# gopro/cineform-sdk

Measured on AMD Instinct MI355X. Metric: 1080p YUY2 encode+decode fps, higher is better.
Workload: dtype int16

## Files before the change

cineform-sdk_amd/csrc/cfhd_device.hip:

```cpp
#include "cfhd_device.h"
#include "cfhd_kernels.h"
#include "cfhd_collect_kernels.h"
#include <hip/hip_runtime.h>
#include <string.h>
#include <stddef.h>
#include <vector>
#include <stdlib.h>
#include <stdio.h>
#include <mutex>
#include <thread>
#include <atomic>
#include <string>
#include <utility>

namespace cfhd {

namespace {
std::string g_err_text; std::mutex g_err_mutex;
thread_local std::string t_err_copy;
struct ErrSlot { ErrSlot &operator=(const char *t) { std::lock_guard<std::mutex> l(g_err_mutex); g_err_text = t; return *this; } } g_err;
std::once_flag g_init_once;
int g_init_rc = -1;
int g_device = 0;

// ... 564 lines not shown
		if (pitch == in_pitch_) memcpy(dst + off, src + (size_t)r0 * pitch, bytes);
		else for (int r = r0; r < r1; r++) memcpy(dst + (size_t)r * in_pitch_, src + (size_t)r * pitch, (size_t)in_pitch_);
		HIPCHK(hipMemcpyAsync(d_in_ + frame_bytes_ * i + off, dst + off, bytes, hipMemcpyHostToDevice, (hipStream_t)stream_));
	}
	return 0;
}

int EncodeBatch::upload_frames(const void *frames, size_t frame_stride, int pitch)
{
	(void)hipSetDevice(device_);
	if (!frames) return -1;
	if (plan_.pixel_kind == PIX_AV28 && pitch >= 0) pitch = in_pitch_;
	if (pitch == in_pitch_ && frame_stride == frame_bytes_ && plan_.pixel_kind != PIX_BYR4 && plan_.pixel_kind != PIX_BYR5 && host_buffer_is_registered(frames, frame_bytes_ * (size_t)n_)) {
		HIPCHK(hipMemcpyAsync(d_in_, frames, frame_bytes_ * (size_t)n_, hipMemcpyHostToDevice, (hipStream_t)stream_));
		return 0;
	}
	if (n_ > 8 && pitch >= in_pitch_ && plan_.pixel_kind != PIX_BYR4 && plan_.pixel_kind != PIX_BYR5 && !host_buffer_is_registered(frames, 1)) {
		const int nt = n_ < 8 ? n_ : 8;
		std::atomic<int> next(0);
		auto work = [&] {
			for (int i; (i = next.fetch_add(1)) < n_;) {
				const uint8_t *src = (const uint8_t *)frames + frame_stride * (size_t)i; uint8_t *dst = h_in_ + frame_bytes_ * (size_t)i;
				if (pitch == in_pitch_) memcpy(dst, src, frame_bytes_);
				else for (int r = 0; r < in_rows_; r++) memcpy(dst + (size_t)r * in_pitch_, src + (size_t)r * pitch, (size_t)in_pitch_);
			}
		};
		std::vector<std::thread> pool;
		for (int k = 1; k < nt; k++) pool.emplace_back(work);
		work();
		for (auto &t : pool) t.join();
		HIPCHK(hipMemcpyAsync(d_in_, h_in_, frame_bytes_ * (size_t)n_, hipMemcpyHostToDevice, (hipStream_t)stream_));
		return 0;
	}
	for (int i = 0; i < n_; i++) { const int rc = upload_frame(i, (const uint8_t *)frames + frame_stride * (size_t)i, pitch); if (rc) return rc; }
	return 0;
}

static double frames_1080p_equivalent(const FramePlan &plan, int frames) { return (double)frames * plan.width * plan.height / (1920.0 * 1080.0); }
static int shape_override(const char *name)
{
	const char *e = getenv(name);
	return !e ? 0 : (strcmp(e, "tile") == 0 ? 1 : (strcmp(e, "strip") == 0 ? 2 : 0));
}
static int active_frames(int active, int n) { return active > 0 && active < n ? active : n; }
static bool planes_as_strips(const FramePlan &plan, int lv , int frames)
{
	const int forced = shape_override("CFHD_AMD_PLANES");
	double samples = 0.0;
	for (int c = 0; c < plan.num_channels; c++) samples += (double)plan.ch[c].width * plan.ch[c].height;
	if (forced == 1 || (forced == 0 && frames * samples / (2.0 * 1920.0 * 1080.0) < 160.0)) return false;
	for (int c = 0; c < plan.num_channels; c++) {
		const BandDesc &b = plan.ch[c].band[lv][0];
		if (b.width % dev::SBLK || plan.ch[c].band[lv - 1][0].width != 2 * b.width || plan.ch[c].band[lv - 1][0].height != 2 * b.height ||
		    (plan.ch[c].band[lv - 1][0].pitch & 7) || (b.pitch & 7)) return false;
	}
	return true;
}
template <typename F> static void for_channel_runs(const FramePlan &plan, int lv, F f)
{
	for (int c0 = 0; c0 < plan.num_channels;) {
		int nc = 1;
		while (c0 + nc < plan.num_channels && plan.ch[c0 + nc].band[lv][0].width == plan.ch[c0].band[lv][0].width &&
		       plan.ch[c0 + nc].band[lv][0].height == plan.ch[c0].band[lv][0].height) nc++;
		const BandDesc &b = plan.ch[c0].band[lv][0];
		int glog = 0; while ((1 << glog) < b.width / dev::SBLK) glog++;
		const int nblk = b.width / dev::SBLK, nseg = nblk > 64 ? (nblk + dev::PLSTEP - 1) / dev::PLSTEP : 1;
		if (nseg > 1) glog = 6;
		f(c0, nc, glog, b, nseg);
		c0 += nc;
	}
}

struct PlaneStrips { int nstrips; unsigned blocks; };
static PlaneStrips plane_strips(int frames, int nc, int glog, int nseg, int band_height)
{
	const int nstrips = (band_height + dev::SRP - 1) / dev::SRP, per_wave = nseg > 1 ? 1 : 64 >> glog, waves = ((frames * nc + per_wave - 1) / per_wave) * nstrips * nseg;
	return { nstrips, (unsigned)((waves + 3) / 4) };
}
static void launch_fwd_plane_tiles(const dev::FwdPlaneJob *jobs, int width, int height, int planes, hipStream_t st) { dev::k_fwd_plane<<<dim3((width / 2 + dev::TW - 1) / dev::TW, (height / 2 + dev::TH - 1) / dev::TH, planes), dev::NTHREADS, 0, st>>>(jobs); }

enum class FwdL1 { Yuv422, Yuv422Strip, Yuv422StripBlocks, Yuv422StripBlocksDense, FrameYuv422, FrameYuv422Strip, Packed16, Packed16Strip, BayerStrip, BayerUnpack, GopPacked16 };
static const char *const kFwdL1Name[] = {"k_fwd_yuv422", "k_fwd_yuv422_strip", "k_fwd_yuv422_strip_blocks", "k_fwd_yuv422_strip_blocks_dense", "k_fwd_frame_yuv422",
                                         "k_fwd_frame_yuv422_strip", "k_fwd_packed16", "k_fwd_packed16_strip", "k_fwd_bayer_strip", "k_unpack_byr4+k_fwd_plane", "k_fwd_gop_packed16"};
static const char *const kFwdPlaneName[2] = {"k_fwd_plane", "k_fwd_plane_strip"};
static_assert(sizeof(kFwdL1Name) / sizeof(*kFwdL1Name) == (size_t)FwdL1::GopPacked16 + 1, "one name per level-1 kernel");
struct ForwardRoute {
	FwdL1 l1; bool strip_planes[2];
	bool block_lists() const { return l1 == FwdL1::Yuv422StripBlocks || l1 == FwdL1::Yuv422StripBlocksDense; }
};
template <typename F> static bool every_frame(int n, F ok) { for (int i = 0; i < n; i++) if (!ok(i)) return false; return true; }

ForwardRoute EncodeBatch::forward_route(bool coeffs_needed, int frames) const
{
	static const int blocks_env = [] { const char *e = getenv("CFHD_AMD_BLOCKS"); return e ? atoi(e) : 1; }();
	const int act = frames, forced = shape_override("CFHD_AMD_FORWARD"), kind = plan_.pixel_kind, nch = plan_.num_channels;
	const EncJobs j = enc_jobs_at(h_jobs_, n_, nch);
	ForwardRoute r;
	for (int lv = 1; lv < 3; lv++) r.strip_planes[lv - 1] = planes_as_strips(plan_, lv, act);
	const bool strips = forced != 1 && (forced != 0 || frames_1080p_equivalent(plan_, act) >= 32.0);
	const bool yuy2 = kind == PIX_YUY2 || kind == PIX_2VUY, bayer = kind == PIX_BYR4 || kind == PIX_BYR5;
	const bool yuv_strips = strips && plan_.encoded_format == ENC_YUV422 && plan_.width % 32 == 0 &&
	                        every_frame(n_, [&](int i) { return !((uintptr_t)j.yuv[i].in & 15) && !(j.yuv[i].in_pitch & 15); });
	if (bayer) {
		const bool ok = strips && kind == PIX_BYR4 && plan_.width % 8 == 0 && nch == 4 &&
		                every_frame(n_, [&](int i) { return !((uintptr_t)j.bayer[i].in & 15) && !((j.bayer[i].in_pitch * 2) & 15) && j.bayer[i].order == j.bayer[0].order; });
		r.l1 = ok ? FwdL1::BayerStrip : FwdL1::BayerUnpack;
	} else if (strips && is_packed16(kind) && plan_.encoded_format != ENC_YUV422 && plan_.width % 8 == 0 && nch >= 3 && every_frame(n_, [&](int i) {
		const dev::FwdPlaneJob &p = j.l1[(size_t)i * nch];
		const uintptr_t frame = (uintptr_t)((const uint16_t *)p.in - packed_word_of_channel(kind, 0));
		return !(frame & 15) && !((p.in_pitch * 2) & 15) && p.layout == dev::FWD_WORDS16 && p.width % 8 == 0; })) r.l1 = FwdL1::Packed16Strip;
	else if (enc_packed16(kind)) r.l1 = FwdL1::Packed16;
	else if (plan_.interlaced) r.l1 = yuv_strips && yuy2 ? FwdL1::FrameYuv422Strip : FwdL1::FrameYuv422;
	else if (!yuv_strips) r.l1 = FwdL1::Yuv422;
	else if (blocks_env && ent_ready_ && ent_.block_slots() && yuy2) r.l1 = coeffs_needed ? FwdL1::Yuv422StripBlocksDense : FwdL1::Yuv422StripBlocks;
	else r.l1 = FwdL1::Yuv422Strip;
	return r;
}

struct FirstLevel {
	int width, height, frames;
	const dev::FwdYuvJob *yuv; const dev::FwdPlaneJob *l1; const dev::BayerJob *bayer;
	int nch, pixel_kind;
	int luma_tiles, chroma_tiles;
};
static int launch_first_level(FwdL1 k, const FirstLevel &g, hipStream_t st)
{
	static_assert(sizeof(dev::FwdFrameJob) == sizeof(dev::FwdYuvJob) && offsetof(dev::FwdFrameJob, q) == offsetof(dev::FwdYuvJob, q), "the two level-1 jobs share one table");
	const int hw = g.width / 2, hh = g.height / 2, act = g.frames, nch = g.nch;
	const dim3 tiles((hw + dev::TW - 1) / dev::TW, (hh + dev::TH - 1) / dev::TH, act);
	auto strips422 = [&](int rows) { return dim3((g.width / 16 + dev::SSEG - 1) / dev::SSEG, (hh + rows - 1) / rows, act); };
	const int nseg = (g.width / 8 + dev::PSTEP - 1) / dev::PSTEP, nstrips = (hh + dev::PSR - 1) / dev::PSR, waves = act * nseg * nstrips;
	const dev::FwdFrameJob *frame = (const dev::FwdFrameJob *)g.yuv;
	const bool bayer = k == FwdL1::BayerStrip || k == FwdL1::BayerUnpack, planes = bayer || k == FwdL1::Packed16 || k == FwdL1::Packed16Strip || k == FwdL1::GopPacked16;
	if ((planes ? !g.l1 : !g.yuv) || (bayer && !g.bayer)) { g_err = "forward level 1: no job table for the kernel"; return -1; }
	switch (k) {
	case FwdL1::Packed16: dev::k_fwd_packed16<<<dim3(tiles.x * nch, tiles.y, act), dev::NTHREADS, 0, st>>>(g.l1, nch); break;
	case FwdL1::GopPacked16: dev::k_fwd_gop_packed16<<<dim3(g.luma_tiles + 2 * g.chroma_tiles, tiles.y, act), dev::NTHREADS, 0, st>>>(g.l1, g.luma_tiles); break;
	case FwdL1::BayerStrip: dev::k_fwd_bayer_strip<<<(waves + 3) / 4, dev::NTHREADS, 0, st>>>(g.l1, g.bayer, act, nseg, nstrips); break;
	case FwdL1::BayerUnpack:
		dev::k_unpack_byr4<<<dim3((hw + dev::NTHREADS - 1) / dev::NTHREADS, g.height, act), dev::NTHREADS, 0, st>>>(g.bayer);
		launch_fwd_plane_tiles(g.l1, g.width, g.height, act * nch, st);
		break;
	case FwdL1::Packed16Strip:
		if (g.pixel_kind == PIX_RG48) dev::k_fwd_packed16_strip<3, 3><<<dim3((waves + 3) / 4), dev::NTHREADS, 0, st>>>(g.l1, act, nseg, nstrips);
		else if (nch == 4) dev::k_fwd_packed16_strip<4, 4><<<dim3((waves + 3) / 4), dev::NTHREADS, 0, st>>>(g.l1, act, nseg, nstrips);
		else dev::k_fwd_packed16_strip<4, 3><<<dim3((waves + 3) / 4), dev::NTHREADS, 0, st>>>(g.l1, act, nseg, nstrips);
		break;
	case FwdL1::FrameYuv422Strip: dev::k_fwd_frame_yuv422_strip<<<strips422(dev::SRI), dev::NTHREADS, 0, st>>>(frame); break;
	case FwdL1::FrameYuv422: dev::k_fwd_frame_yuv422<<<dim3((hw + dev::FTW - 1) / dev::FTW, (hh + dev::FRW - 1) / dev::FRW, act), dev::NTHREADS, 0, st>>>(frame); break;
	case FwdL1::Yuv422StripBlocksDense: dev::k_fwd_yuv422_strip_blocks_dense<<<strips422(dev::SRF), dev::NTHREADS, 0, st>>>(g.yuv); break;
	case FwdL1::Yuv422StripBlocks: dev::k_fwd_yuv422_strip_blocks<<<strips422(dev::SRF), dev::NTHREADS, 0, st>>>(g.yuv); break;
	case FwdL1::Yuv422Strip: dev::k_fwd_yuv422_strip<<<strips422(dev::SRF), dev::NTHREADS, 0, st>>>(g.yuv); break;
	case FwdL1::Yuv422: dev::k_fwd_yuv422<<<tiles, dev::NTHREADS, 0, st>>>(g.yuv); break;
	}
	return 0;
}

const char *EncodeBatch::level_kernel(int level, bool coeffs_needed) const
{
	const ForwardRoute r = forward_route(coeffs_needed, active_frames(active_, n_));
	return level > 0 ? kFwdPlaneName[r.strip_planes[level - 1]] : kFwdL1Name[(int)r.l1];
}

int EncodeBatch::launch_forward(bool coeffs_needed, int first, int count)
{
	if (!count) count = active_frames(active_, n_);
	if (first < 0 || count < 1 || first + count > n_) return -1;
	(void)hipSetDevice(device_);
	const ForwardRoute r = forward_route(coeffs_needed, count);
	if (ent_ready_) ent_.set_block_lists(r.block_lists());
	int rc = sync_jobs();
	if (rc) return rc;
	hipStream_t st = (hipStream_t)stream_;
	const int nch = plan_.num_channels;
	const int act = count;
	EncJobs j = enc_jobs_at(d_jobs_, n_, nch);
	if (j.yuv) j.yuv += first;
	if (j.bayer) j.bayer += first;
	if (j.l1) j.l1 += (size_t)first * nch;
	j.l2 += (size_t)first * nch; j.l3 += (size_t)first * nch;
	(void)hipGetLastError();
	timed_ = true;
	HIPCHK(hipEventRecord((hipEvent_t)ev0_, st));
	rc = launch_first_level(r.l1, { plan_.width, plan_.height, act, j.yuv, j.l1, j.bayer, nch, plan_.pixel_kind, 0, 0 }, st);
	if (rc) return rc;
	for (int lv = 1; lv < 3; lv++) {
		HIPCHK(hipEventRecord((hipEvent_t)evl_[lv - 1], st));
		const BandDesc &src = plan_.ch[0].band[lv - 1][0];
		const dev::FwdPlaneJob *jobs = lv == 1 ? j.l2 : j.l3;
		if (r.strip_planes[lv - 1]) {
			for_channel_runs(plan_, lv, [&](int c0, int nc, int glog, const BandDesc &b, int nseg) {
				const PlaneStrips g = plane_strips(act, nc, glog, nseg, b.height);
				dev::k_fwd_plane_strip<<<g.blocks, dev::NTHREADS, 0, st>>>(jobs, act, nch, c0, nc, glog, g.nstrips, 2 * b.width, 2 * b.height, nseg);
			});
			continue;
		}
		launch_fwd_plane_tiles(jobs, src.width, src.height, act * nch, st);
	}
	HIPCHK(hipGetLastError());
	HIPCHK(hipEventRecord((hipEvent_t)ev1_, st));
	return 0;
}

int EncodeBatch::download_coeffs()
{
	(void)hipSetDevice(device_);
	HIPCHK(hipMemcpy2DAsync(h_coeff_, (size_t)plan_.final_elems * 2, d_coeff_, (size_t)plan_.coeff_elems * 2,
	                        (size_t)plan_.final_elems * 2, n_, hipMemcpyDeviceToHost, (hipStream_t)stream_));
	return 0;
}

int EncodeBatch::wait()
{
	(void)hipSetDevice(device_);
	HIPCHK(hipStreamSynchronize((hipStream_t)stream_));
	collect_.resolve();
	float ms = 0;
	if (!timed_) return 0;
	timed_ = false;
	if (hipEventElapsedTime(&ms, (hipEvent_t)ev0_, (hipEvent_t)ev1_) == hipSuccess) kernel_ms_ = ms;
	if (hipEventElapsedTime(&ms, (hipEvent_t)ev0_, (hipEvent_t)evl_[0]) == hipSuccess) level_ms_[0] = ms;
	if (hipEventElapsedTime(&ms, (hipEvent_t)evl_[0], (hipEvent_t)evl_[1]) == hipSuccess) level_ms_[1] = ms;
	if (hipEventElapsedTime(&ms, (hipEvent_t)evl_[1], (hipEvent_t)ev1_) == hipSuccess) level_ms_[2] = ms;
	return 0;
}

static OutputRoute output_route(int encoded_format, int kind, bool half, bool interlaced)
{
	OutputRoute r; r.work = kind; r.lowpass_kind = kind;
	const bool yuv8 = kind == PIX_YUY2 || kind == PIX_2VUY, rgb32 = kind == PIX_BGRA || kind == PIX_BGRa, rgb16 = is_packed16(kind), rgb8 = dec_rgb8(kind), rgb10 = dec_rgb10(kind);
	auto refuse = [&r](const char *text) { r.refusal = text; return r; };
	static const char *const not_served = "output format not supported by the GPU path yet";
	if (kind == PIX_BYR4) {
		if (encoded_format != ENC_BAYER || half) return refuse("BYR4 output: Bayer samples, full resolution");
		r.jobs = OutJobs::Planes16; r.work = PIX_RG48; r.convert = OutConvert::Byr4;
		return r;
	}
	if (encoded_format == ENC_YUV422) {
		if (!yuv8 && kind != PIX_YU64 && kind != PIX_V210 && !rgb8 && !rgb16) return refuse(not_served);
		if (kind == PIX_V210) { r.work = PIX_YU64; r.convert = OutConvert::V210; r.width_multiple = 6; r.width_refusal = "v210 output: widths that are multiples of 6"; }
		if (half) {
			r.jobs = OutJobs::HalfYuv;
			if (rgb8 || rgb16) { r.half_mode = kind == PIX_RG24 ? 0 : (kind == PIX_RG48 ? 2 : (kind == PIX_B64A ? 3 : 1)); r.bottom_up = kind == PIX_BGRA; }
			if (rgb32) { r.width_multiple = 16; r.width_refusal = "BGRA / BGRa output of 4:2:2 samples: half widths that are multiples of 16"; }
			return r;
		}
		if (yuv8) return r;
		if (rgb32 && !interlaced) return r;
		r.work = PIX_YU64;
		r.jobs = interlaced && (rgb16 || rgb32) ? OutJobs::Yuv : OutJobs::Planes16;
		if (kind == PIX_RG24) r.convert = OutConvert::Rgb24;
		if (rgb16 || rgb32) { r.convert = OutConvert::Rgb16; r.rgb16_mode = kind == PIX_BGRA ? 3 : (kind == PIX_BGRa ? 2 : (kind == PIX_B64A ? 1 : 0)); }
		return r;
	}
	const bool rgb = encoded_format == ENC_RGB444, rgba = encoded_format == ENC_RGBA4444;
	if (!((rgb16 && (rgb || rgba)) || (rgb8 && (rgb || (rgba && kind != PIX_RG24))) || (rgb10 && rgb))) return refuse(not_served);
	if (!half) { r.jobs = OutJobs::Planes16; return r; }
	r.jobs = OutJobs::HalfPacked;
	if (rgb8 || rgb10 || (kind == PIX_B64A && rgb)) {
		r.half_mode = rgb8 ? 1 : (rgb10 ? 2 : 3); r.half_bytes = rgb8 ? rgb8_bytes(kind) : 0;
		r.bottom_up = kind == PIX_RG24 || kind == PIX_BGRA; r.big_endian = kind == PIX_R210 || kind == PIX_DPX0;
	}
	return r;
}

static void fill_half_yuv_job(dev::HalfYuvJob &hj, const Level1 &l, const OutputRoute &r, int rows, int matrix, uint8_t *out, int out_pitch)
{
// ... 764 lines not shown
		g = e;
	}
	return 0;
}

int GopBatch::upload_frame(int f, const void *frame, int pitch)
{
	(void)hipSetDevice(device_);
	if (decode_ || f < 0 || f >= 2 * n_) return -1;
	const uint8_t *src = (const uint8_t *)frame;
	const bool av28 = plan_.pixel_kind == PIX_AV28;
	if (pitch < 0) { src += (ptrdiff_t)(rows_ - 1) * pitch; pitch = -pitch; }
	uint8_t *dst = h_frames_ + frame_bytes_ * f;
	if (pitch == pitch_ || av28) memcpy(dst, src, frame_bytes_);
	else for (int r = 0; r < rows_; r++) memcpy(dst + (size_t)r * pitch_, src + (size_t)r * pitch, (size_t)pitch_);
	HIPCHK(hipMemcpyAsync(d_frames_ + frame_bytes_ * f, dst, frame_bytes_, hipMemcpyHostToDevice, (hipStream_t)stream_));
	return 0;
}

int GopBatch::upload_frame_device(int f, const void *d_frame, int pitch)
{
	(void)hipSetDevice(device_);
	if (decode_ || f < 0 || f >= 2 * n_ || !d_frame) return -1;
	const uint8_t *src = (const uint8_t *)d_frame;
	if (pitch < 0) { src += (ptrdiff_t)(rows_ - 1) * pitch; pitch = -pitch; }
	if (plan_.pixel_kind == PIX_AV28) {
		HIPCHK(hipMemcpyAsync(d_frames_ + frame_bytes_ * f, src, frame_bytes_, hipMemcpyDeviceToDevice, (hipStream_t)stream_));
		return 0;
	}
	if (pitch < pitch_) return -1;
	HIPCHK(hipMemcpy2DAsync(d_frames_ + frame_bytes_ * f, (size_t)pitch_, src, (size_t)pitch, (size_t)pitch_, (size_t)rows_, hipMemcpyDeviceToDevice, (hipStream_t)stream_));
	return 0;
}

int GopBatch::upload_frames_device_planar(int first, int count, const void *d_frames, size_t frame_stride, int row_pitch, int layout)
{
	(void)hipSetDevice(device_);
	if (decode_) return -1;
	return collect_planar_frames(plan_.pixel_kind, d_frames_, frame_bytes_, pitch_, plan_.width, rows_, 2 * n_, first, count, d_frames, frame_stride, row_pitch, layout, stream_, collect_);
}

int GopBatch::download_input_frame(int f, void *out, int pitch)
{
	(void)hipSetDevice(device_);
	const size_t row = pitch_ ? (size_t)pitch_ : frame_bytes_, nrows = pitch_ ? (size_t)rows_ : 1;
	if (decode_ || f < 0 || f >= 2 * n_ || !out || pitch < 0 || (size_t)pitch < row) return -1;
	HIPCHK(hipMemcpy2DAsync(out, (size_t)pitch, d_frames_ + frame_bytes_ * f, row, row, nrows, hipMemcpyDeviceToHost, (hipStream_t)stream_));
	HIPCHK(hipStreamSynchronize((hipStream_t)stream_));
	return 0;
}

int GopBatch::upload_frames(const void *frames, size_t frame_stride, int pitch)
{
	(void)hipSetDevice(device_);
	if (decode_ || !frames || pitch <= 0) return -1;
	const size_t total = 2 * (size_t)n_ * frame_bytes_;
	const bool av28 = plan_.pixel_kind == PIX_AV28;
	if ((pitch == pitch_ || av28) && frame_stride == frame_bytes_ && host_buffer_is_registered(frames, total)) {
		HIPCHK(hipMemcpyAsync(d_frames_, frames, total, hipMemcpyHostToDevice, (hipStream_t)stream_));
		return 0;
	}
	for (int f = 0; f < 2 * n_; f++) {
		const uint8_t *src = (const uint8_t *)frames + frame_stride * (size_t)f;
		uint8_t *dst = h_frames_ + frame_bytes_ * f;
		if (pitch == pitch_ || av28) memcpy(dst, src, frame_bytes_);
		else for (int r = 0; r < rows_; r++) memcpy(dst + (size_t)r * pitch_, src + (size_t)r * pitch, (size_t)(pitch < pitch_ ? pitch : pitch_));
	}
	HIPCHK(hipMemcpyAsync(d_frames_, h_frames_, total, hipMemcpyHostToDevice, (hipStream_t)stream_));
	return 0;
}

int GopBatch::launch_forward(int first, int count)
{
	if (first < 0 || count < 1 || first + count > n_) return -1;
	(void)hipSetDevice(device_);
	hipStream_t st = (hipStream_t)stream_;
	const int rcj = sync_jobs();
	if (rcj) return rcj;
	GopJobs j = gop_jobs_at(d_jobs_, n_);
	j.yuv += 2 * first; j.fl1 += 6 * first; j.temp += 3 * first; j.mid += 6 * first; j.top += 3 * first; j.tq += 3 * first;
	(void)hipGetLastError();
	if (timed_) HIPCHK(hipEventRecord((hipEvent_t)ev_[0], st));
	const int luma_tiles = (plan_.ch[0].width / 2 + dev::TW - 1) / dev::TW, chroma_tiles = (plan_.ch[1].width / 2 + dev::TW - 1) / dev::TW;
	const int rc = launch_first_level(forward_route(), { plan_.width, plan_.height, 2 * count, j.yuv, j.fl1, nullptr, 3, plan_.pixel_kind, luma_tiles, chroma_tiles }, st);
	if (rc) return rc;
	if (timed_) HIPCHK(hipEventRecord((hipEvent_t)ev_[1], st));
	const GopWavelet &t = plan_.ch[0].w[2];
	dev::k_gop_temporal_fwd<<<dim3((unsigned)((t.pitch * t.height / 2 + dev::NTHREADS - 1) / dev::NTHREADS), 3 * count), dev::NTHREADS, 0, st>>>(j.temp);
	launch_fwd_plane_tiles(j.mid, t.width, t.height, 6 * count, st);
	if (!decode_ && gop_temporal_lowpass_is_coded(plan_)) {
		const GopWavelet &w3 = plan_.ch[0].w[3];
		dev::k_gop_quant_lowpass<<<dim3((unsigned)((w3.pitch * w3.height / 2 + dev::NTHREADS - 1) / dev::NTHREADS), 3 * count), dev::NTHREADS, 0, st>>>(j.tq);
	}
	if (timed_) HIPCHK(hipEventRecord((hipEvent_t)ev_[2], st));
	const GopWavelet &m = plan_.ch[0].w[4];
	launch_fwd_plane_tiles(j.top, m.width, m.height, 3 * count, st);
	HIPCHK(hipGetLastError());
	if (timed_) { HIPCHK(hipEventRecord((hipEvent_t)ev_[3], st)); launched_ = true; }
	return 0;
}

int GopBatch::download_coeffs()
{
	(void)hipSetDevice(device_);
	HIPCHK(hipMemcpyAsync(h_coeff_, d_coeff_, plan_.coeff_elems * 2, hipMemcpyDeviceToHost, (hipStream_t)stream_));
	return 0;
}

int GopBatch::launch_inverse(uint32_t dither_seed, bool coeffs_on_device)
{
	(void)hipSetDevice(device_);
	hipStream_t st = (hipStream_t)stream_;
	if (jobs_dirty_) { HIPCHK(hipMemcpyAsync(d_jobs_, h_jobs_, jobs_bytes_, hipMemcpyHostToDevice, st)); jobs_dirty_ = false; }
	if (!coeffs_on_device) HIPCHK(hipMemcpyAsync(d_coeff_, h_coeff_, plan_.coeff_elems * 2, hipMemcpyHostToDevice, st));
	if (!coeffs_on_device && n_ != 1) return -1;
	GopJobs j = gop_jobs_at(d_jobs_, n_);
	const int ng = active_groups();
	(void)hipGetLastError();
	if (timed_) HIPCHK(hipEventRecord((hipEvent_t)ev_[0], st));
	const GopWavelet &top = plan_.ch[0].w[5], &mid = plan_.ch[0].w[4], &t = plan_.ch[0].w[2], &l1 = plan_.ch[0].w[0];
	dev::k_inv_plane<<<dim3((top.width + dev::ITW - 1) / dev::ITW, (top.height + dev::ITH - 1) / dev::ITH, 3 * ng), dev::NTHREADS, 0, st>>>(j.itop);
	if (timed_) HIPCHK(hipEventRecord((hipEvent_t)ev_[1], st));
	dev::k_inv_plane<<<dim3((mid.width + dev::ITW - 1) / dev::ITW, (mid.height + dev::ITH - 1) / dev::ITH, 6 * ng), dev::NTHREADS, 0, st>>>(j.imid);
	dev::k_gop_temporal_inv<<<dim3((unsigned)((t.pitch * t.height / 2 + dev::NTHREADS - 1) / dev::NTHREADS), 3 * ng), dev::NTHREADS, 0, st>>>(j.temp);
	if (timed_) HIPCHK(hipEventRecord((hipEvent_t)ev_[2], st));
	const GopRoute r = route();
	const int rc = launch_last_level(r.l1, { l1.width, l1.height, rows_, 2 * ng, plan_.interlaced, j.iyuv, j.l1, j.half, nullptr, 3, dec_words_per_position(PIX_YU64, 3) }, dither_seed, st);
	if (rc) return rc;
	auto convert = [&](int f, int nf, size_t step, int m) {
		launch_convert(r.out, d_tmp_ + tmp_frame_bytes_ * f, tmp_pitch_, tmp_frame_bytes_ * step, d_frames_ + frame_bytes_ * f, pitch_, frame_bytes_ * step, half_ ? plan_.width / 2 : plan_.width, rows_, 0, nf, m,
		               dither_seed + 0x9E3779B9u * (uint32_t)f, nullptr, st);
	};
	if (matrix_ == 0 || r.out.convert == OutConvert::V210) convert(0, 2 * ng, 1, 0); else { convert(0, ng, 2, matrix_); convert(1, ng, 2, 0); }
	HIPCHK(hipGetLastError());
	if (timed_) { HIPCHK(hipEventRecord((hipEvent_t)ev_[3], st)); launched_ = true; }
	return 0;
}

int GopBatch::download_frame(int f, void *, int)
{
	(void)hipSetDevice(device_);
	if (!decode_ || f < 0 || f >= 2 * n_) return -1;
	HIPCHK(hipMemcpyAsync(h_frames_ + frame_bytes_ * f, d_frames_ + frame_bytes_ * f, frame_bytes_, hipMemcpyDeviceToHost, (hipStream_t)stream_));
	return 0;
}

int GopBatch::download_frames(void *out, size_t, int pitch)
{
	(void)hipSetDevice(device_);
	if (!decode_ || !out || pitch <= 0) return -1;
	HIPCHK(hipMemcpyAsync(h_frames_, d_frames_, 2 * (size_t)active_groups() * frame_bytes_, hipMemcpyDeviceToHost, (hipStream_t)stream_));
	return 0;
}

int GopBatch::finish_frame(int f, void *out, int pitch)
{
	if (!decode_ || f < 0 || f >= 2 * n_) return -1;
	const uint8_t *src = h_frames_ + frame_bytes_ * f;
	if (pitch == pitch_) memcpy(out, src, frame_bytes_);
	else for (int r = 0; r < rows_; r++) memcpy((uint8_t *)out + (ptrdiff_t)r * pitch, src + (size_t)r * pitch_, (size_t)pitch_);
	return 0;
}

int GopBatch::wait()
{
	(void)hipSetDevice(device_);
	HIPCHK(hipStreamSynchronize((hipStream_t)stream_));
// ... 6 lines not shown
```

cineform-sdk_amd/csrc/cfhd_kernels.h:

```cpp
#pragma once
#include <stdint.h>
#include <cfhd_gfx950.h>

namespace cfhd {
namespace dev {

enum { TW = 64, TH = 16, ROWS = 2 * TH + 4, NTHREADS = 256, NSTAGE = (ROWS * (TW + 4) + NTHREADS - 1) / NTHREADS };

struct QuantParam { int mid; unsigned mult; int divisor; };

struct FwdPlaneJob {
	const int16_t *in; int in_pitch;
	int width, height;
	int prescale;
	int16_t *out[4]; int out_pitch;
	QuantParam q[4];
	int xstride, shift, display_height;
	int compand;
	int layout, tail_from;
	const uint16_t *curve;
};
enum FwdLayout { FWD_WORDS16 = 0, FWD_V210_Y = 1, FWD_V210_CR = 2, FWD_V210_CB = 3, FWD_BYTES8_BOTTOM_UP = 4, FWD_BYTES8_TOP_DOWN = 5, FWD_RGB10 = 6, FWD_RGB16_AS_422 = 7,
                 FWD_BYTES8_AS_422_BOTTOM_UP = 8, FWD_BYTES8_AS_422_TOP_DOWN = 9, FWD_BAYER_BYR4 = 10, FWD_BAYER_BYR5 = 11,
                 FWD_AVID_BYTES8 = 12, FWD_AVID_WORDS16 = 13, FWD_AVID_S214 = 14, FWD_AVID_2_8 = 15 };
// ... 1086 lines not shown
		const int jn = more ? inv_window_first_row(r + 1, h) : j;
		const bool advance = jn != j;
		StripRow nll = ll2, nlh = lh2, nhl = hl, nhh = hh;
		if (!LATE_LOADS) {
			if (advance) { nll = strip_load(pLL + (size_t)(jn + 2) * pitch); nlh = LOAD_LH(jn + 2); }
			if (more) { nhl = LOAD_HL(r + 1); nhh = LOAD_HH(r + 1); }
		}
		const int pos = r == 0 ? 0 : (r == h - 1 ? 2 : 1);
		uint32_t Lv[2][4], Hv[2][4];
		if (pos == 1) {
#pragma unroll
			for (int d = 0; d < 4; d++) {
				inv_vert_pk(ll0.d[d], ll1.d[d], ll2.d[d], hl.d[d], 1, Lv[0][d], Lv[1][d]);
				inv_vert_pk(lh0.d[d], lh1.d[d], lh2.d[d], hh.d[d], 1, Hv[0][d], Hv[1][d]);
			}
		} else {
#pragma unroll
			for (int d = 0; d < 4; d++) {
				inv_vert_pk(ll0.d[d], ll1.d[d], ll2.d[d], hl.d[d], pos, Lv[0][d], Lv[1][d]);
				inv_vert_pk(lh0.d[d], lh1.d[d], lh2.d[d], hh.d[d], pos, Hv[0][d], Hv[1][d]);
			}
		}
		uint32_t (*rowbuf)[SROW / 4] = s_rows[s & 1];
#pragma unroll
		for (int par = 0; par < 2; par++) {
			const int orow = 2 * r + par;
			const uint32_t prev = __shfl(Lv[par][3], lane - 1), next = __shfl(Lv[par][0], lane + 1);
			const uint32_t X = sh >= 2 ? rotr32(dither_word(seed, orow, dgroup), drot) : 0u;
			uint32_t out[4];
			strip_row_to8(Lv[par], Hv[par], prev, next, first, last, sh + 1, X, out);
			if (stores) {
				uint32_t *dst = &rowbuf[par][lds_at];
#pragma unroll
				for (int d = 0; d < 4; d++) dst[d] = out[d];
			}
		}
		__syncthreads();
		if (tid < nquads) {
#pragma unroll
			for (int par = 0; par < 2; par++) {
				const int orow = 2 * r + par;
				if (orow >= display_height) continue;
				const uint32_t *row = rowbuf[par];
				const uint32_t y0 = row[2 * tid], y1 = row[2 * tid + 1], vv = row[v_base + tid], uu = row[u_base + tid];
				const uint32_t uv01 = byte_perm(vv, uu, 0x05010400u), uv23 = byte_perm(vv, uu, 0x07030602u);
				uint4 q;
				if (uyvy) {
					q.x = byte_perm(uv01, y0, 0x01050004u); q.y = byte_perm(uv01, y0, 0x03070206u);
					q.z = byte_perm(uv23, y1, 0x01050004u); q.w = byte_perm(uv23, y1, 0x03070206u);
				} else {
					q.x = byte_perm(uv01, y0, 0x05010400u); q.y = byte_perm(uv01, y0, 0x07030602u);
					q.z = byte_perm(uv23, y1, 0x05010400u); q.w = byte_perm(uv23, y1, 0x07030602u);
				}
				*(uint4 *)(out_base + (size_t)orow * out_pitch + 32 * (size_t)seg_first + 16 * (size_t)tid) = q;
			}
		}
		if (LATE_LOADS) {
			if (advance) { nll = strip_load(pLL + (size_t)(jn + 2) * pitch); nlh = LOAD_LH(jn + 2); }
			if (more) { nhl = LOAD_HL(r + 1); nhh = LOAD_HH(r + 1); }
		}
		if (advance) { ll0 = ll1; ll1 = ll2; ll2 = nll; lh0 = lh1; lh1 = lh2; lh2 = nlh; j = jn; }
		hl = nhl; hh = nhh;
	}
#undef pLL
#undef pLH
#undef pHL
#undef pHH
#undef LOAD_LH
#undef LOAD_HL
#undef LOAD_HH
}
__global__ void __launch_bounds__(NTHREADS) k_inv_yuv422_strip(const InvYuvJob *jobs, uint32_t launch_seed) { inv_yuv422_strip<SR, true>(jobs, launch_seed); }
__global__ void __launch_bounds__(NTHREADS) k_inv_yuv422_strip_blocks(const InvYuvJob *jobs, uint32_t launch_seed) { inv_yuv422_strip<SR, true, true>(jobs, launch_seed); }

enum { SRF = 32, SFPLANE = 512 };

__device__ __forceinline__ void strip_fwd_row(const uint32_t (&p)[8], uint32_t prev, uint32_t next, bool first, bool last, uint32_t (&L)[4], uint32_t (&H)[4], int prescale = 0)
{
	const uint32_t ext[10] = { prev, p[0], p[1], p[2], p[3], p[4], p[5], p[6], p[7], next };
#pragma unroll
	for (int m = 0; m < 4; m++) horiz_pair(&ext[2 * m], 0u, prescale, first && m == 0, false, last && m == 3, L[m], H[m]);
}

enum { FWD_LATE_LOADS = 2 };
struct FwdStrip {
	uint32_t LW[6][4], HW[6][4];
	cfhd_u4 raw[2][2];
};

__device__ __forceinline__ void strip_fwd_fetch(FwdStrip &st, const FwdYuvJob &job, const uint8_t *in, int y)
{
#pragma unroll
	for (int k = 0; k < 2; k++) {
		if (y + k < job.display_height) { const uint8_t *p = in + (size_t)(y + k) * job.in_pitch; st.raw[k][0] = CFHD_LDG128(p); st.raw[k][1] = CFHD_LDG128(p + 16); }
		else { cfhd_u4 g; g.x = g.y = g.z = g.w = 0x80808080u; st.raw[k][0] = g; st.raw[k][1] = g; }
	}
}

template <int SLOT>
__device__ __forceinline__ void strip_fwd_push(FwdStrip &st, const FwdYuvJob &job, const uint8_t *in, uint32_t (*buf)[2][SFPLANE], int y, bool prefetch,
                                               bool luma, int comp, int lds_write_at, int lds_read_at, int lane, bool first, bool last, int shift, int ysh0, uint32_t usel, uint32_t vsel)
{
	uint32_t p[2][8];
	if (luma) {
		if (FWD_LATE_LOADS == 2) strip_fwd_fetch(st, job, in, y);
		uint32_t a[2][8];
#pragma unroll
		for (int k = 0; k < 2; k++) {
			a[k][0] = st.raw[k][0].x; a[k][1] = st.raw[k][0].y; a[k][2] = st.raw[k][0].z; a[k][3] = st.raw[k][0].w;
			a[k][4] = st.raw[k][1].x; a[k][5] = st.raw[k][1].y; a[k][6] = st.raw[k][1].z; a[k][7] = st.raw[k][1].w;
		}
		if (prefetch && !FWD_LATE_LOADS) strip_fwd_fetch(st, job, in, y + 2);
#pragma unroll
		for (int k = 0; k < 2; k++) {
#pragma unroll
			for (int i = 0; i < 8; i++) p[k][i] = ((a[k][i] >> ysh0) & 0x00ff00ffu) << shift;
			if (lds_write_at >= 0) {
#pragma unroll
				for (int i = 0; i < 4; i++) {
					buf[k][0][lds_write_at + i] = byte_perm(a[k][2 * i + 1], a[k][2 * i], vsel) << shift;
					buf[k][1][lds_write_at + i] = byte_perm(a[k][2 * i + 1], a[k][2 * i], usel) << shift;
				}
			}
		}
	}
	__syncthreads();
	if (!luma) {
#pragma unroll
		for (int k = 0; k < 2; k++) {
#pragma unroll
			for (int i = 0; i < 8; i++) p[k][i] = buf[k][comp - 1][lds_read_at + i < 0 ? 0 : lds_read_at + i];
		}
	}
#pragma unroll
	for (int k = 0; k < 2; k++) {
		const uint32_t prev = __shfl(p[k][7], lane - 1), next = __shfl(p[k][0], lane + 1);
		strip_fwd_row(p[k], prev, next, first, last, st.LW[SLOT + k], st.HW[SLOT + k]);
	}
	if (luma && prefetch && FWD_LATE_LOADS == 1) strip_fwd_fetch(st, job, in, y + 2);
}

template <int ROWS_PER_STRIP, bool BLOCKS = false, bool DENSE = true>
__device__ __forceinline__ void fwd_yuv422_strip(const FwdYuvJob *jobs)
{
	const TileId tile = xcd_tile();
	__shared__ FwdYuvJob s_job;
	stage_job(&s_job, &jobs[tile.z]);
	const FwdYuvJob &job = s_job;
	__shared__ uint32_t s_pairs[2][2][2][SFPLANE];
	const int W = job.width, H = job.height, HH = H >> 1;
	const int r0 = tile.y * ROWS_PER_STRIP;
	const int tid = threadIdx.x, wave = tid >> 6, lane = tid & 63;
	const bool luma = wave < 2;
	const int comp = luma ? 0 : wave - 1;
	const QuantParam q_lh = wave_uniform_quant(job.q[comp][1]), q_hl = wave_uniform_quant(job.q[comp][2]), q_hh = wave_uniform_quant(job.q[comp][3]);
	const int nblk = luma ? W / 16 : W / 32;
	const int seg_first = tile.x * SSEG;
	const int base = luma ? seg_first + SLUMA_STEP * wave : seg_first >> 1;
	const int want = base - 1 + lane;
	const int blk = want < 0 ? 0 : (want < nblk ? want : nblk - 1);
	const bool stores = lane >= 1 && lane <= SLUMA_STEP && want < nblk;
	const bool first = blk == 0, last = blk == nblk - 1;
	const int lds_write_at = (luma && want >= 0 && want < nblk && (wave == 0 ? lane <= SLUMA_STEP : lane >= 1)) ? 4 * (want - seg_first + 1) : -1;
	const int lds_read_at = 8 * lane - 4;
	if (r0 >= HH) return;
	const int r1 = r0 + ROWS_PER_STRIP < HH ? r0 + ROWS_PER_STRIP : HH;
	const int shift = job.shift;
	const int ysh0 = job.uyvy ? 8 : 0, ub = job.uyvy ? 0 : 1, vb = job.uyvy ? 2 : 3;
	const uint32_t usel = (uint32_t)ub | 0x0c00u | ((uint32_t)(4 + ub) << 16) | 0x0c000000u;
	const uint32_t vsel = (uint32_t)vb | 0x0c00u | ((uint32_t)(4 + vb) << 16) | 0x0c000000u;
	const uint8_t *in = job.in + 32 * (size_t)blk;
	static_assert(SLUMA_STEP == FWD_CHUNK_BLOCKS, "a chunk is what one wave stores of a band row");
	const int chunks_per_row = BLOCKS ? wave_uniform((nblk + FWD_CHUNK_BLOCKS - 1) / FWD_CHUNK_BLOCKS) : 0, chunk = BLOCKS ? wave_uniform(base / FWD_CHUNK_BLOCKS) : 0;
	uint4 *slot0[3]; unsigned long long *mask0[3];
	const int opitch = wave_uniform(job.out_pitch[comp]), pitch8 = opitch >> 3;
	int16_t *outp[4];
#pragma unroll
	for (int b = 0; b < 4; b++) outp[b] = wave_uniform_ptr(job.out[comp][b]);
	if (BLOCKS) {
#pragma unroll
		for (int b = 1; b < 4; b++) {
			slot0[b - 1] = wave_uniform_ptr(job.lists.blocks + (size_t)(job.out[comp][b] - job.lists.base) / 8 + (size_t)(FWD_CHUNK_BLOCKS * chunk));
			mask0[b - 1] = wave_uniform_ptr(job.lists.masks + job.lists.mask_base[comp][b] + chunk);
		}
	}
	FwdStrip st;
	int wtop = window_first_row(r0, HH, H);
	const int lastrow = window_first_row(r1 - 1, HH, H) + 5;
	int t = 0;
#define CFHD_PUSH(SLOT, Y) strip_fwd_push<SLOT>(st, job, in, s_pairs[t & 1], (Y), (Y) + 2 <= lastrow, luma, comp, lds_write_at, lds_read_at, lane, first, last, shift, ysh0, usel, vsel); t++
	if (luma && FWD_LATE_LOADS != 2) strip_fwd_fetch(st, job, in, wtop);
	CFHD_PUSH(0, wtop); CFHD_PUSH(2, wtop + 2); CFHD_PUSH(4, wtop + 4);
	auto band_row = [&](const int r, const int pos) {
		uint32_t o[4][4];
#pragma unroll
		for (int d = 0; d < 4; d++) {
			uint32_t ll, lh, hl, hh;
			if (pos == 1) {
				ll = pk_adds(st.LW[2][d], st.LW[3][d]); hl = pk_hp_mid(st.LW[0][d], st.LW[1][d], st.LW[2][d], st.LW[3][d], st.LW[4][d], st.LW[5][d]);
				lh = pk_adds(st.HW[2][d], st.HW[3][d]); hh = pk_hp_mid(st.HW[0][d], st.HW[1][d], st.HW[2][d], st.HW[3][d], st.HW[4][d], st.HW[5][d]);
			} else {
				int res[4][2];
#pragma unroll
				for (int e = 0; e < 2; e++) {
					int a[6], b[6];
#pragma unroll
					for (int k = 0; k < 6; k++) { a[k] = e ? hi16(st.LW[k][d]) : lo16(st.LW[k][d]); b[k] = e ? hi16(st.HW[k][d]) : lo16(st.HW[k][d]); }
					if (pos == 0) {
						res[0][e] = sat16(a[0] + a[1]); res[2][e] = hp_first(a[0], a[1], a[2], a[3], a[4], a[5]);
						res[1][e] = sat16(b[0] + b[1]); res[3][e] = hp_first(b[0], b[1], b[2], b[3], b[4], b[5]);
					} else {
						res[0][e] = sat16(a[4] + a[5]); res[2][e] = hp_last(a[0], a[1], a[2], a[3], a[4], a[5]);
						res[1][e] = sat16(b[4] + b[5]); res[3][e] = hp_last(b[0], b[1], b[2], b[3], b[4], b[5]);
					}
				}
				ll = pack16(res[0][0], res[0][1]); lh = pack16(res[1][0], res[1][1]); hl = pack16(res[2][0], res[2][1]); hh = pack16(res[3][0], res[3][1]);
			}
			o[0][d] = ll; o[1][d] = pk_quantize(lh, q_lh);
			o[2][d] = pk_quantize(hl, q_hl); o[3][d] = pk_quantize(hh, q_hh);
		}
		if (BLOCKS) {
#pragma unroll
			for (int b = 1; b < 4; b++) {
				const bool nz = stores && (o[b][0] | o[b][1] | o[b][2] | o[b][3]) != 0u;
				const unsigned long long m = __ballot(nz);
				uint4 *rowslots = wave_uniform_ptr(slot0[b - 1] + (size_t)(r * pitch8));
				if (nz) store_u32x4_global(rowslots + wave_mbcnt(m), o[b][0], o[b][1], o[b][2], o[b][3]);
				if (lane == 0 && chunk < chunks_per_row) mask0[b - 1][r * chunks_per_row] = m >> 1;
			}
		}
		if (stores) {
#pragma unroll
			for (int b = 0; b < 4; b++) {
				if (b && BLOCKS && !DENSE) continue;
				store_u32x4_global(outp[b] + (uint32_t)(r * opitch + SBLK * blk), o[b][0], o[b][1], o[b][2], o[b][3]);
			}
		}
	};
	auto window_down = [&]() {
#pragma unroll
		for (int k = 0; k < 4; k++) {
#pragma unroll
			for (int d = 0; d < 4; d++) { st.LW[k][d] = st.LW[k + 2][d]; st.HW[k][d] = st.HW[k + 2][d]; }
		}
	};
	auto any_row = [&](const int r) {
		const int need = window_first_row(r, HH, H);
		if (need != wtop) { window_down(); wtop = need; CFHD_PUSH(4, wtop + 4); }
		band_row(r, r == 0 ? 0 : (r == HH - 1 ? 2 : 1));
	};
	int r = r0;
	for (; r < r1 && (r == r0 || r < 2); r++) any_row(r);
	const int mid_end = r1 < HH - 1 ? r1 : HH - 1;
#define CFHD_MID_ROW(R) window_down(); wtop += 2; CFHD_PUSH(4, wtop + 4); band_row((R), 1)
	for (; r + 3 <= mid_end; r += 3) { CFHD_MID_ROW(r); CFHD_MID_ROW(r + 1); CFHD_MID_ROW(r + 2); }
	for (; r < mid_end; r++) { CFHD_MID_ROW(r); }
#undef CFHD_MID_ROW
	for (; r < r1; r++) any_row(r);
#undef CFHD_PUSH
}
__global__ void __launch_bounds__(NTHREADS) k_fwd_yuv422_strip(const FwdYuvJob *jobs) { fwd_yuv422_strip<SRF>(jobs); }
__global__ void __launch_bounds__(NTHREADS) __attribute__((amdgpu_waves_per_eu(4, 4))) k_fwd_yuv422_strip_blocks(const FwdYuvJob *jobs) { fwd_yuv422_strip<SRF, true, false>(jobs); }
__global__ void __launch_bounds__(NTHREADS) k_fwd_yuv422_strip_blocks_dense(const FwdYuvJob *jobs) { fwd_yuv422_strip<SRF, true, true>(jobs); }

enum { SRP = 16 };

struct StripWho { int job; int blk; bool stores; int strip; };
enum { PLSTEP = 62 };
__device__ __forceinline__ StripWho strip_who(int nframes, int nch, int c0, int nc, int glog, int nstrips, int nblk, bool *wave_idle, int nseg = 1)
{
	const int lane = threadIdx.x & 63, gwave = (int)blockIdx.x * (NTHREADS / 64) + (int)(threadIdx.x >> 6);
	const bool segments = nseg > 1;
	const int per_wave = segments ? 1 : 64 >> glog, sub = segments ? 0 : lane >> glog;
	const int strip = gwave % nstrips, rest = gwave / nstrips, seg = segments ? rest % nseg : 0;
	const int b = segments ? seg * PLSTEP - 1 + lane : (lane & ((1 << glog) - 1));
	const int first_sel = (segments ? rest / nseg : rest) * per_wave, nsel = nframes * nc;
	*wave_idle = first_sel >= nsel;
	int sel = first_sel + sub;
	const bool job_ok = sel < nsel;
	if (!job_ok) sel = nsel - 1;
	StripWho w;
	w.job = (sel / nc) * nch + c0 + sel % nc;
	w.stores = job_ok && b >= 0 && b < nblk && (!segments || (lane >= 1 && lane <= PLSTEP));
	w.blk = b < 0 ? 0 : (b < nblk ? b : nblk - 1);
	w.strip = strip;
	return w;
}

__global__ void __launch_bounds__(NTHREADS) k_inv_plane_strip(const InvPlaneJob *jobs, int nframes, int nch, int c0, int nc, int glog, int nstrips, int w, int h, int nseg)
{
	const int lane = threadIdx.x & 63;
	const int nblk = w / SBLK;
	bool idle;
	const StripWho who = strip_who(nframes, nch, c0, nc, glog, nstrips, nblk, &idle, nseg);
	if (idle) return;
	const InvPlaneJob *job = &jobs[who.job];
	const int blk = who.blk, pitch = job->band_pitch, descale = job->descale;
	const bool first = blk == 0, last = blk == nblk - 1;
	const int16_t *pLL = job->band[0] + SBLK * blk, *pLH = job->band[1] + SBLK * blk, *pHL = job->band[2] + SBLK * blk, *pHH = job->band[3] + SBLK * blk;
	int16_t *out = job->out + 2 * SBLK * blk;
	const int out_pitch = job->out_pitch;
	const int r0 = who.strip * SRP;
	const int nrows = h - r0 < SRP ? h - r0 : SRP;
	int j = inv_window_first_row(r0, h);
	StripRow ll0 = strip_load(pLL + (size_t)j * pitch), ll1 = strip_load(pLL + (size_t)(j + 1) * pitch), ll2 = strip_load(pLL + (size_t)(j + 2) * pitch);
	StripRow lh0 = strip_load(pLH + (size_t)j * pitch), lh1 = strip_load(pLH + (size_t)(j + 1) * pitch), lh2 = strip_load(pLH + (size_t)(j + 2) * pitch);
	StripRow hl = strip_load(pHL + (size_t)r0 * pitch), hh = strip_load(pHH + (size_t)r0 * pitch);
	for (int s = 0; s < nrows; s++) {
		const int r = r0 + s;
		const bool more = s + 1 < nrows;
		const int jn = more ? inv_window_first_row(r + 1, h) : j;
		const bool advance = jn != j;
		StripRow nll = ll2, nlh = lh2, nhl = hl, nhh = hh;
		const int pos = r == 0 ? 0 : (r == h - 1 ? 2 : 1);
		uint32_t Lv[2][4], Hv[2][4];
		if (pos == 1) {
#pragma unroll
			for (int d = 0; d < 4; d++) {
				inv_vert_pk(ll0.d[d], ll1.d[d], ll2.d[d], hl.d[d], 1, Lv[0][d], Lv[1][d]);
				inv_vert_pk(lh0.d[d], lh1.d[d], lh2.d[d], hh.d[d], 1, Hv[0][d], Hv[1][d]);
			}
		} else {
#pragma unroll
			for (int d = 0; d < 4; d++) {
				inv_vert_pk(ll0.d[d], ll1.d[d], ll2.d[d], hl.d[d], pos, Lv[0][d], Lv[1][d]);
				inv_vert_pk(lh0.d[d], lh1.d[d], lh2.d[d], hh.d[d], pos, Hv[0][d], Hv[1][d]);
			}
		}
#pragma unroll
		for (int par = 0; par < 2; par++) {
			const uint32_t (&L)[4] = Lv[par];
			const uint32_t (&H)[4] = Hv[par];
			const uint32_t prev = __shfl(L[3], lane - 1), next = __shfl(L[0], lane + 1);
			const uint32_t ext[6] = { prev, L[0], L[1], L[2], L[3], next };
			uint32_t o[8];
#pragma unroll
			for (int d = 0; d < 4; d++) {
				const uint32_t dm = ext[d], d0 = ext[d + 1], dp = ext[d + 2];
				uint32_t even, odd;
				inv_horiz_pk((dm >> 16) | (d0 << 16), d0, (d0 >> 16) | (dp << 16), H[d], even, odd);
				if (descale) { even = pk_adds(even, even); odd = pk_adds(odd, odd); }
				else { even = pk_sra(even, 1); odd = pk_sra(odd, 1); }
				o[2 * d] = pk_lolo(even, odd); o[2 * d + 1] = pk_hihi(even, odd);
			}
			if (first) {
				const int l[6] = { 0, 0, lo16(L[0]), hi16(L[0]), lo16(L[1]), hi16(L[1]) };
// ... 1326 lines not shown
```

Baseline: 67670.

## Compute strip forward wavelet with sum/difference factoring instead of full 6-tap filters

Rewrites the level-1 YUV422 strip forward transform to compute the highpass filter from pairwise sums and differences. The horizontal highpass becomes (next sum - prev sum + 4)>>3 plus the difference, and the vertical pass stores row-pair sums and differences so the band step needs only a subtract, shift and add. This removes redundant packed adds and multiply-like tap work in the hot loop. The new path is used only when every frame's shift is in 0..3, where the refactoring is assumed exact. Otherwise new _taps kernel variants keep the original tap arithmetic, at the cost of three extra kernel instantiations.

```diff
diff --git a/cineform-sdk_amd/csrc/cfhd_device.hip b/cineform-sdk_amd/csrc/cfhd_device.hip
--- a/cineform-sdk_amd/csrc/cfhd_device.hip
+++ b/cineform-sdk_amd/csrc/cfhd_device.hip
@@ -670,10 +670,21 @@
 enum class FwdL1 { Yuv422, Yuv422Strip, Yuv422StripBlocks, Yuv422StripBlocksDense, FrameYuv422, FrameYuv422Strip, Packed16, Packed16Strip, BayerStrip, BayerUnpack, GopPacked16 };
 static const char *const kFwdL1Name[] = {"k_fwd_yuv422", "k_fwd_yuv422_strip", "k_fwd_yuv422_strip_blocks", "k_fwd_yuv422_strip_blocks_dense", "k_fwd_frame_yuv422",
                                          "k_fwd_frame_yuv422_strip", "k_fwd_packed16", "k_fwd_packed16_strip", "k_fwd_bayer_strip", "k_unpack_byr4+k_fwd_plane", "k_fwd_gop_packed16"};
+static const char *fwd_l1_name(FwdL1 k, bool taps)
+{
+	if (taps) switch (k) {
+	case FwdL1::Yuv422Strip: return "k_fwd_yuv422_strip_taps";
+	case FwdL1::Yuv422StripBlocks: return "k_fwd_yuv422_strip_blocks_taps";
+	case FwdL1::Yuv422StripBlocksDense: return "k_fwd_yuv422_strip_blocks_dense_taps";
+	default: break;
+	}
+	return kFwdL1Name[(int)k];
+}
 static const char *const kFwdPlaneName[2] = {"k_fwd_plane", "k_fwd_plane_strip"};
 static_assert(sizeof(kFwdL1Name) / sizeof(*kFwdL1Name) == (size_t)FwdL1::GopPacked16 + 1, "one name per level-1 kernel");
 struct ForwardRoute {
 	FwdL1 l1; bool strip_planes[2];
+	bool taps;
 	bool block_lists() const { return l1 == FwdL1::Yuv422StripBlocks || l1 == FwdL1::Yuv422StripBlocksDense; }
 };
 template <typename F> static bool every_frame(int n, F ok) { for (int i = 0; i < n; i++) if (!ok(i)) return false; return true; }
@@ -689,6 +700,7 @@
 	const bool yuy2 = kind == PIX_YUY2 || kind == PIX_2VUY, bayer = kind == PIX_BYR4 || kind == PIX_BYR5;
 	const bool yuv_strips = strips && plan_.encoded_format == ENC_YUV422 && plan_.width % 32 == 0 &&
 	                        every_frame(n_, [&](int i) { return !((uintptr_t)j.yuv[i].in & 15) && !(j.yuv[i].in_pitch & 15); });
+	r.taps = yuv_strips && !every_frame(n_, [&](int i) { return dev::fwd_sums_exact(j.yuv[i].shift); });
 	if (bayer) {
 		const bool ok = strips && kind == PIX_BYR4 && plan_.width % 8 == 0 && nch == 4 &&
 		                every_frame(n_, [&](int i) { return !((uintptr_t)j.bayer[i].in & 15) && !((j.bayer[i].in_pitch * 2) & 15) && j.bayer[i].order == j.bayer[0].order; });
@@ -710,6 +722,7 @@
 	const dev::FwdYuvJob *yuv; const dev::FwdPlaneJob *l1; const dev::BayerJob *bayer;
 	int nch, pixel_kind;
 	int luma_tiles, chroma_tiles;
+	bool taps;
 };
 static int launch_first_level(FwdL1 k, const FirstLevel &g, hipStream_t st)
 {
@@ -736,9 +749,18 @@
 		break;
 	case FwdL1::FrameYuv422Strip: dev::k_fwd_frame_yuv422_strip<<<strips422(dev::SRI), dev::NTHREADS, 0, st>>>(frame); break;
 	case FwdL1::FrameYuv422: dev::k_fwd_frame_yuv422<<<dim3((hw + dev::FTW - 1) / dev::FTW, (hh + dev::FRW - 1) / dev::FRW, act), dev::NTHREADS, 0, st>>>(frame); break;
-	case FwdL1::Yuv422StripBlocksDense: dev::k_fwd_yuv422_strip_blocks_dense<<<strips422(dev::SRF), dev::NTHREADS, 0, st>>>(g.yuv); break;
-	case FwdL1::Yuv422StripBlocks: dev::k_fwd_yuv422_strip_blocks<<<strips422(dev::SRF), dev::NTHREADS, 0, st>>>(g.yuv); break;
-	case FwdL1::Yuv422Strip: dev::k_fwd_yuv422_strip<<<strips422(dev::SRF), dev::NTHREADS, 0, st>>>(g.yuv); break;
+	case FwdL1::Yuv422StripBlocksDense:
+		if (g.taps) dev::k_fwd_yuv422_strip_blocks_dense_taps<<<strips422(dev::SRF), dev::NTHREADS, 0, st>>>(g.yuv);
+		else dev::k_fwd_yuv422_strip_blocks_dense<<<strips422(dev::SRF), dev::NTHREADS, 0, st>>>(g.yuv);
+		break;
+	case FwdL1::Yuv422StripBlocks:
+		if (g.taps) dev::k_fwd_yuv422_strip_blocks_taps<<<strips422(dev::SRF), dev::NTHREADS, 0, st>>>(g.yuv);
+		else dev::k_fwd_yuv422_strip_blocks<<<strips422(dev::SRF), dev::NTHREADS, 0, st>>>(g.yuv);
+		break;
+	case FwdL1::Yuv422Strip:
+		if (g.taps) dev::k_fwd_yuv422_strip_taps<<<strips422(dev::SRF), dev::NTHREADS, 0, st>>>(g.yuv);
+		else dev::k_fwd_yuv422_strip<<<strips422(dev::SRF), dev::NTHREADS, 0, st>>>(g.yuv);
+		break;
 	case FwdL1::Yuv422: dev::k_fwd_yuv422<<<tiles, dev::NTHREADS, 0, st>>>(g.yuv); break;
 	}
 	return 0;
@@ -747,7 +769,7 @@
 const char *EncodeBatch::level_kernel(int level, bool coeffs_needed) const
 {
 	const ForwardRoute r = forward_route(coeffs_needed, active_frames(active_, n_));
-	return level > 0 ? kFwdPlaneName[r.strip_planes[level - 1]] : kFwdL1Name[(int)r.l1];
+	return level > 0 ? kFwdPlaneName[r.strip_planes[level - 1]] : fwd_l1_name(r.l1, r.taps);
 }
 
 int EncodeBatch::launch_forward(bool coeffs_needed, int first, int count)
@@ -770,7 +792,7 @@
 	(void)hipGetLastError();
 	timed_ = true;
 	HIPCHK(hipEventRecord((hipEvent_t)ev0_, st));
-	rc = launch_first_level(r.l1, { plan_.width, plan_.height, act, j.yuv, j.l1, j.bayer, nch, plan_.pixel_kind, 0, 0 }, st);
+	rc = launch_first_level(r.l1, { plan_.width, plan_.height, act, j.yuv, j.l1, j.bayer, nch, plan_.pixel_kind, 0, 0, r.taps }, st);
 	if (rc) return rc;
 	for (int lv = 1; lv < 3; lv++) {
 		HIPCHK(hipEventRecord((hipEvent_t)evl_[lv - 1], st));
@@ -1701,7 +1723,7 @@
 	(void)hipGetLastError();
 	if (timed_) HIPCHK(hipEventRecord((hipEvent_t)ev_[0], st));
 	const int luma_tiles = (plan_.ch[0].width / 2 + dev::TW - 1) / dev::TW, chroma_tiles = (plan_.ch[1].width / 2 + dev::TW - 1) / dev::TW;
-	const int rc = launch_first_level(forward_route(), { plan_.width, plan_.height, 2 * count, j.yuv, j.fl1, nullptr, 3, plan_.pixel_kind, luma_tiles, chroma_tiles }, st);
+	const int rc = launch_first_level(forward_route(), { plan_.width, plan_.height, 2 * count, j.yuv, j.fl1, nullptr, 3, plan_.pixel_kind, luma_tiles, chroma_tiles, false }, st);
 	if (rc) return rc;
 	if (timed_) HIPCHK(hipEventRecord((hipEvent_t)ev_[1], st));
 	const GopWavelet &t = plan_.ch[0].w[2];
diff --git a/cineform-sdk_amd/csrc/cfhd_kernels.h b/cineform-sdk_amd/csrc/cfhd_kernels.h
--- a/cineform-sdk_amd/csrc/cfhd_kernels.h
+++ b/cineform-sdk_amd/csrc/cfhd_kernels.h
@@ -1192,6 +1192,25 @@
 	for (int m = 0; m < 4; m++) horiz_pair(&ext[2 * m], 0u, prescale, first && m == 0, false, last && m == 3, L[m], H[m]);
 }
 
+inline bool fwd_sums_exact(int shift) { return shift >= 0 && shift <= 3; }
+__device__ __forceinline__ void strip_fwd_row_sums(const uint32_t (&p)[8], int lane, bool first, bool last, uint32_t (&L)[4], uint32_t (&H)[4])
+{
+	uint32_t D[4];
+#pragma unroll
+	for (int m = 0; m < 4; m++) {
+		const uint32_t e = pk_lolo(p[2 * m], p[2 * m + 1]), o = pk_hihi(p[2 * m], p[2 * m + 1]);
+		L[m] = pk_adds(e, o); D[m] = pk_subs(e, o);
+	}
+	const uint32_t ext[6] = { __shfl(L[3], lane - 1), L[0], L[1], L[2], L[3], __shfl(L[0], lane + 1) };
+	uint32_t A[5];
+#pragma unroll
+	for (int k = 0; k < 5; k++) A[k] = (ext[k] >> 16) | (ext[k + 1] << 16);
+#pragma unroll
+	for (int m = 0; m < 4; m++) H[m] = pk_adds(pk_sra(pk_adds(pk_subs(A[m + 1], A[m]), pk_set(4)), 3), D[m]);
+	if (first) H[0] = pack16(hp_first(lo16(p[0]), hi16(p[0]), lo16(p[1]), hi16(p[1]), lo16(p[2]), hi16(p[2])), hi16(H[0]));
+	if (last) H[3] = pack16(lo16(H[3]), hp_last(lo16(p[5]), hi16(p[5]), lo16(p[6]), hi16(p[6]), lo16(p[7]), hi16(p[7])));
+}
+
 enum { FWD_LATE_LOADS = 2 };
 struct FwdStrip {
 	uint32_t LW[6][4], HW[6][4];
@@ -1207,7 +1226,7 @@
 	}
 }
 
-template <int SLOT>
+template <int SLOT, bool SUMS>
 __device__ __forceinline__ void strip_fwd_push(FwdStrip &st, const FwdYuvJob &job, const uint8_t *in, uint32_t (*buf)[2][SFPLANE], int y, bool prefetch,
                                                bool luma, int comp, int lds_write_at, int lds_read_at, int lane, bool first, bool last, int shift, int ysh0, uint32_t usel, uint32_t vsel)
 {
@@ -1244,13 +1263,21 @@
 	}
 #pragma unroll
 	for (int k = 0; k < 2; k++) {
-		const uint32_t prev = __shfl(p[k][7], lane - 1), next = __shfl(p[k][0], lane + 1);
-		strip_fwd_row(p[k], prev, next, first, last, st.LW[SLOT + k], st.HW[SLOT + k]);
+		if (SUMS) strip_fwd_row_sums(p[k], lane, first, last, st.LW[SLOT + k], st.HW[SLOT + k]);
+		else strip_fwd_row(p[k], __shfl(p[k][7], lane - 1), __shfl(p[k][0], lane + 1), first, last, st.LW[SLOT + k], st.HW[SLOT + k]);
+	}
+	if (SUMS) {
+#pragma unroll
+		for (int d = 0; d < 4; d++) {
+			const uint32_t l0 = st.LW[SLOT][d], l1 = st.LW[SLOT + 1][d], h0 = st.HW[SLOT][d], h1 = st.HW[SLOT + 1][d];
+			st.LW[SLOT][d] = pk_adds(l0, l1); st.LW[SLOT + 1][d] = pk_subs(l0, l1);
+			st.HW[SLOT][d] = pk_adds(h0, h1); st.HW[SLOT + 1][d] = pk_subs(h0, h1);
+		}
 	}
 	if (luma && prefetch && FWD_LATE_LOADS == 1) strip_fwd_fetch(st, job, in, y + 2);
 }
 
-template <int ROWS_PER_STRIP, bool BLOCKS = false, bool DENSE = true>
+template <int ROWS_PER_STRIP, bool BLOCKS = false, bool DENSE = true, bool SUMS = true>
 __device__ __forceinline__ void fwd_yuv422_strip(const FwdYuvJob *jobs)
 {
 	const TileId tile = xcd_tile();
@@ -1298,7 +1325,7 @@
 	int wtop = window_first_row(r0, HH, H);
 	const int lastrow = window_first_row(r1 - 1, HH, H) + 5;
 	int t = 0;
-#define CFHD_PUSH(SLOT, Y) strip_fwd_push<SLOT>(st, job, in, s_pairs[t & 1], (Y), (Y) + 2 <= lastrow, luma, comp, lds_write_at, lds_read_at, lane, first, last, shift, ysh0, usel, vsel); t++
+#define CFHD_PUSH(SLOT, Y) strip_fwd_push<SLOT, SUMS>(st, job, in, s_pairs[t & 1], (Y), (Y) + 2 <= lastrow, luma, comp, lds_write_at, lds_read_at, lane, first, last, shift, ysh0, usel, vsel); t++
 	if (luma && FWD_LATE_LOADS != 2) strip_fwd_fetch(st, job, in, wtop);
 	CFHD_PUSH(0, wtop); CFHD_PUSH(2, wtop + 2); CFHD_PUSH(4, wtop + 4);
 	auto band_row = [&](const int r, const int pos) {
@@ -1306,9 +1333,28 @@
 #pragma unroll
 		for (int d = 0; d < 4; d++) {
 			uint32_t ll, lh, hl, hh;
-			if (pos == 1) {
+			if (pos == 1 && SUMS) {
+				ll = st.LW[2][d]; hl = pk_adds(pk_sra(pk_adds(pk_subs(st.LW[4][d], st.LW[0][d]), pk_set(4)), 3), st.LW[3][d]);
+				lh = st.HW[2][d]; hh = pk_adds(pk_sra(pk_adds(pk_subs(st.HW[4][d], st.HW[0][d]), pk_set(4)), 3), st.HW[3][d]);
+			} else if (pos == 1) {
 				ll = pk_adds(st.LW[2][d], st.LW[3][d]); hl = pk_hp_mid(st.LW[0][d], st.LW[1][d], st.LW[2][d], st.LW[3][d], st.LW[4][d], st.LW[5][d]);
 				lh = pk_adds(st.HW[2][d], st.HW[3][d]); hh = pk_hp_mid(st.HW[0][d], st.HW[1][d], st.HW[2][d], st.HW[3][d], st.HW[4][d], st.HW[5][d]);
+			} else if (SUMS) {
+				int res[4][2];
+#pragma unroll
+				for (int e = 0; e < 2; e++) {
+					int a[6], b[6];
+#pragma unroll
+					for (int k = 0; k < 6; k++) { a[k] = e ? hi16(st.LW[k][d]) : lo16(st.LW[k][d]); b[k] = e ? hi16(st.HW[k][d]) : lo16(st.HW[k][d]); }
+					if (pos == 0) {
+						res[0][e] = a[0]; res[2][e] = sat16((-3 * a[0] + 8 * a[1] + 4 * a[2] - a[4] + 4) >> 3);
+						res[1][e] = b[0]; res[3][e] = sat16((-3 * b[0] + 8 * b[1] + 4 * b[2] - b[4] + 4) >> 3);
+					} else {
+						res[0][e] = a[4]; res[2][e] = sat16((3 * a[4] + 8 * a[5] - 4 * a[2] + a[0] + 4) >> 3);
+						res[1][e] = b[4]; res[3][e] = sat16((3 * b[4] + 8 * b[5] - 4 * b[2] + b[0] + 4) >> 3);
+					}
+				}
+				ll = pack16(res[0][0], res[0][1]); lh = pack16(res[1][0], res[1][1]); hl = pack16(res[2][0], res[2][1]); hh = pack16(res[3][0], res[3][1]);
 			} else {
 				int res[4][2];
 #pragma unroll
@@ -1372,6 +1418,9 @@
 __global__ void __launch_bounds__(NTHREADS) k_fwd_yuv422_strip(const FwdYuvJob *jobs) { fwd_yuv422_strip<SRF>(jobs); }
 __global__ void __launch_bounds__(NTHREADS) __attribute__((amdgpu_waves_per_eu(4, 4))) k_fwd_yuv422_strip_blocks(const FwdYuvJob *jobs) { fwd_yuv422_strip<SRF, true, false>(jobs); }
 __global__ void __launch_bounds__(NTHREADS) k_fwd_yuv422_strip_blocks_dense(const FwdYuvJob *jobs) { fwd_yuv422_strip<SRF, true, true>(jobs); }
+__global__ void __launch_bounds__(NTHREADS) k_fwd_yuv422_strip_taps(const FwdYuvJob *jobs) { fwd_yuv422_strip<SRF, false, true, false>(jobs); }
+__global__ void __launch_bounds__(NTHREADS) k_fwd_yuv422_strip_blocks_taps(const FwdYuvJob *jobs) { fwd_yuv422_strip<SRF, true, false, false>(jobs); }
+__global__ void __launch_bounds__(NTHREADS) k_fwd_yuv422_strip_blocks_dense_taps(const FwdYuvJob *jobs) { fwd_yuv422_strip<SRF, true, true, false>(jobs); }
 
 enum { SRP = 16 };
 
```

Result: no change. 68070, median of 6 (+0.6%).
